# diffqc/dqc

Hardware: AMD Instinct MI355X
Metric: SCF iterations/sec (Fock build + XC grid) per GPU, cc-pVDZ 20-atom (higher is better)
Workload: dtype f64

## Files before the change

dqc_amd/csrc/jk.hip:

```cpp
#include <cstdlib>

#include "common.hpp"

namespace dqc {

DQC_DEV void decode_tri(long long t, int &a, int &b) {
    long long r = (long long)((sqrt(8.0 * (double)t + 1.0) - 1.0) * 0.5);
    while (r * (r + 1) / 2 > t) r--;
    while ((r + 1) * (r + 2) / 2 <= t) r++;
    a = (int)r;
    b = (int)(t - r * (r + 1) / 2);
}

DQC_DEV void tile_load_patch(const double *__restrict__ tiles, int IJ, int KL, int I, int J, int K, int L, int r0, int c0, double2 &a0, double2 &b0, double2 &a1, double2 &b1, double2 &a2,
                             double2 &b2, double2 &a3, double2 &b3, const TileLay &ly) {
    const bool dr = I == J, dc = K == L;
    const double *tp = tiles + tile_base(I, J, K, KL, ly);
    const bool trunc = I == ly.last && ly.wl < 8;
    if (!dr && !dc) {
        if (trunc && r0 >= 8 * ly.wl) {
            a0 = b0 = a1 = b1 = a2 = b2 = a3 = b3 = make_double2(0.0, 0.0);
            return;
        }
        const double *q = tp + r0 * 64 + c0;
        a0 = *reinterpret_cast<const double2 *>(q);       b0 = *reinterpret_cast<const double2 *>(q + 2);
        a1 = *reinterpret_cast<const double2 *>(q + 64);  b1 = *reinterpret_cast<const double2 *>(q + 66);
        a2 = *reinterpret_cast<const double2 *>(q + 128); b2 = *reinterpret_cast<const double2 *>(q + 130);
        a3 = *reinterpret_cast<const double2 *>(q + 192); b3 = *reinterpret_cast<const double2 *>(q + 194);
        return;
    }
    const int il = r0 >> 3, j0 = r0 & 7, kl = c0 >> 3, l0 = c0 & 7;
    const double2 z2 = make_double2(0.0, 0.0);
    const bool ok0 = !trunc || (dr ? max(il, j0) < ly.wl : il < ly.wl), ok1 = !trunc || (dr ? max(il, j0 + 1) < ly.wl : il < ly.wl);
    const bool ok2 = !trunc || (dr ? max(il, j0 + 2) < ly.wl : il < ly.wl), ok3 = !trunc || (dr ? max(il, j0 + 3) < ly.wl : il < ly.wl);
    if (!dc) {
        const double *q0 = tp + tile_pidx(true, il, j0) * 64 + c0, *q1 = tp + tile_pidx(true, il, j0 + 1) * 64 + c0;
        const double *q2 = tp + tile_pidx(true, il, j0 + 2) * 64 + c0, *q3 = tp + tile_pidx(true, il, j0 + 3) * 64 + c0;
        a0 = b0 = a1 = b1 = a2 = b2 = a3 = b3 = z2;
        if (ok0) { a0 = *reinterpret_cast<const double2 *>(q0); b0 = *reinterpret_cast<const double2 *>(q0 + 2); }
        if (ok1) { a1 = *reinterpret_cast<const double2 *>(q1); b1 = *reinterpret_cast<const double2 *>(q1 + 2); }
        if (ok2) { a2 = *reinterpret_cast<const double2 *>(q2); b2 = *reinterpret_cast<const double2 *>(q2 + 2); }
        if (ok3) { a3 = *reinterpret_cast<const double2 *>(q3); b3 = *reinterpret_cast<const double2 *>(q3 + 2); }
        return;
    }
    const int C = 36;
    const int pc0 = tile_pidx(dc, kl, l0), pc1 = tile_pidx(dc, kl, l0 + 1), pc2 = tile_pidx(dc, kl, l0 + 2), pc3 = tile_pidx(dc, kl, l0 + 3);
    const double *q0 = tp + tile_pidx(dr, il, j0) * C, *q1 = tp + tile_pidx(dr, il, j0 + 1) * C;
    const double *q2 = tp + tile_pidx(dr, il, j0 + 2) * C, *q3 = tp + tile_pidx(dr, il, j0 + 3) * C;
    a0 = b0 = a1 = b1 = a2 = b2 = a3 = b3 = z2;
    if (ok0) { a0 = make_double2(q0[pc0], q0[pc1]); b0 = make_double2(q0[pc2], q0[pc3]); }
    if (ok1) { a1 = make_double2(q1[pc0], q1[pc1]); b1 = make_double2(q1[pc2], q1[pc3]); }
    if (ok2) { a2 = make_double2(q2[pc0], q2[pc1]); b2 = make_double2(q2[pc2], q2[pc3]); }
    if (ok3) { a3 = make_double2(q3[pc0], q3[pc1]); b3 = make_double2(q3[pc2], q3[pc3]); }
}

__global__ void jk_prep_kernel(double *__restrict__ work, const double *__restrict__ dm, int nao, int npad, int with_k) {
    const size_t n2 = (size_t)npad * npad;
    for (size_t e = (size_t)blockIdx.x * blockDim.x + threadIdx.x; e < n2; e += (size_t)gridDim.x * blockDim.x) {
        const int i = e / npad, j = e % npad;
        double v = 0.0;
        if (i < nao && j < nao) v = 0.5 * (dm[(size_t)i * nao + j] + dm[(size_t)j * nao + i]);
        work[e] = v;
        work[n2 + e] = 0.0;
        if (with_k) work[2 * n2 + e] = 0.0;
    }
}

__global__ void jk_finish_kernel(double *__restrict__ J, double *__restrict__ K, const double *__restrict__ work,
                                 int nao, int npad, const double *__restrict__ dscp) {
    const double dsc = dscp ? *dscp : 0.0;
    const size_t n2 = (size_t)npad * npad;
    const size_t tot = (size_t)nao * nao;
    for (size_t e = (size_t)blockIdx.x * blockDim.x + threadIdx.x; e < tot; e += (size_t)gridDim.x * blockDim.x) {
        const int i = e / nao, j = e % nao;
        J[e] = det_value(work[n2 + (size_t)i * npad + j], dsc) + det_value(work[n2 + (size_t)j * npad + i], dsc);
        if (K) K[e] = det_value(work[2 * n2 + (size_t)i * npad + j], dsc) + det_value(work[2 * n2 + (size_t)j * npad + i], dsc);
    }
}

__global__ __launch_bounds__(256) void jk_det_scale_kernel(double *__restrict__ slot, const double *__restrict__ dms, int nmat,
                                                           size_t n2, const double *__restrict__ tiles, int nao) {
    __shared__ double red[256];
    const int t = threadIdx.x;
    double smax = 0.0;
    for (int q = 0; q < nmat; q++) {
        double sacc = 0.0;
        for (size_t e = t; e < n2; e += 256) sacc += fabs(dms[q * n2 + e]);
        red[t] = sacc;
        __syncthreads();
        for (int o = 128; o > 0; o >>= 1) {
            if (t < o) red[t] += red[t + o];
            __syncthreads();
        }
        smax = fmax(smax, red[0]);
        __syncthreads();
    }
    double g = 0.0;
    for (int i = t; i < nao; i += 256) {
        const long long b = i >> 3, IJ = b * (b + 1) / 2 + b;
        const int pa = tile_pidx(true, i & 7, i & 7);
        g = fmax(g, fabs(tiles[tile_base((int)b, (int)b, (int)b, (int)IJ, TileLay(nao)) + pa * 36 + pa]));
    }
    red[t] = g;
    __syncthreads();
    for (int o = 128; o > 0; o >>= 1) {
        if (t < o) red[t] = fmax(red[t], red[t + o]);
        __syncthreads();
    }
    if (t == 0) {
        const double bound = 2.0 * fmax(red[0], 1e-300) * fmax(smax, 1e-300);
        slot[0] = exp2(floor(61.0 - log2(bound)));
    }
}

template <int NK>
__global__ __launch_bounds__(256, NK ? 3 : 1) void jk_multi_kernel(const double *__restrict__ dscp, const double *__restrict__ tiles,
                                                                   double *__restrict__ work, int npad, long long ntiles, int nj, int nao) {
    const TileLay ly(nao);
    const double dsc = dscp ? *dscp : 0.0;
    constexpr int LDT = 68;
    constexpr int NKD = NK ? NK : 1;
    __shared__ double s_col[2][4][64];
    __shared__ __attribute__((aligned(16))) double s_g[NK ? 64 * LDT : 2];
    __shared__ __attribute__((aligned(16))) double s_d[4][72][NKD];
    const size_t n2 = (size_t)npad * npad;
    const double *Dj = work, *Dk = work + (size_t)nj * n2;
    double *Jacc = work + (size_t)(nj + NK) * n2, *Kacc = Jacc + (size_t)nj * n2;
    const int t = threadIdx.x, lane = t & 63, wave = t >> 6;
    const int r0 = 4 * (t >> 4), c0 = 4 * (t & 15);
    typedef double vd2 __attribute__((ext_vector_type(2)));

    double2 na0, na1, na2, na3, nb0, nb1, nb2, nb3;
#define JKM_LOAD(TT)                                                                     \
    {                                                                                    \
        int ij_, kl_, i_, j_, k_, l_;                                                    \
        decode_tri((TT), ij_, kl_);                                                      \
        decode_tri(ij_, i_, j_);                                                         \
        decode_tri(kl_, k_, l_);                                                         \
        tile_load_patch(tiles, ij_, kl_, i_, j_, k_, l_, r0, c0, na0, nb0, na1, nb1, na2, nb2, na3, nb3, ly); \
    }
    if ((long long)blockIdx.x < ntiles) JKM_LOAD(blockIdx.x)
    for (long long T = blockIdx.x; T < ntiles; T += gridDim.x) {
        int IJ, KL, I, J, K, L;
        decode_tri(T, IJ, KL);
        decode_tri(IJ, I, J);
        decode_tri(KL, K, L);
        const double f = (I == J ? 0.5 : 1.0) * (K == L ? 0.5 : 1.0) * (IJ == KL ? 0.5 : 1.0);
        const int kk = c0 >> 3, l0 = c0 & 7, ii = r0 >> 3, j0 = r0 & 7;
        double g[4][4];
        g[0][0] = na0.x; g[0][1] = na0.y; g[0][2] = nb0.x; g[0][3] = nb0.y;
        g[1][0] = na1.x; g[1][1] = na1.y; g[1][2] = nb1.x; g[1][3] = nb1.y;
        g[2][0] = na2.x; g[2][1] = na2.y; g[2][2] = nb2.x; g[2][3] = nb2.y;
        g[3][0] = na3.x; g[3][1] = na3.y; g[3][2] = nb3.x; g[3][3] = nb3.y;
        if (T + gridDim.x < ntiles) JKM_LOAD(T + gridDim.x)
        if (NK) {
#pragma unroll
            for (int r = 0; r < 4; r++) {
                *reinterpret_cast<double2 *>(&s_g[(r0 + r) * LDT + c0]) = make_double2(g[r][0], g[r][1]);
                *reinterpret_cast<double2 *>(&s_g[(r0 + r) * LDT + c0 + 2]) = make_double2(g[r][2], g[r][3]);
            }
            const int blk = t >> 6, e = t & 63, x = e >> 3, y = e & 7;
            const int R = (blk & 1) ? I : J, Cb = (blk & 2) ? L : K;
#pragma unroll
            for (int q = 0; q < NK; q++) s_d[blk][x * 9 + y][q] = Dk[q * n2 + (size_t)(R * 8 + x) * npad + Cb * 8 + y];
        }
        for (int q = 0; q < nj; q++) {
            const double *dklp = Dj + q * n2 + (size_t)(K * 8 + kk) * npad + L * 8 + l0;
            const double *dijp = Dj + q * n2 + (size_t)(I * 8 + ii) * npad + J * 8 + j0;
            double dkl[4], dij[4];
#pragma unroll
            for (int c = 0; c < 4; c++) { dkl[c] = dklp[c]; dij[c] = dijp[c]; }
            double rs[4] = {0, 0, 0, 0}, cs[4] = {0, 0, 0, 0};
#pragma unroll
            for (int r = 0; r < 4; r++)
#pragma unroll
                for (int c = 0; c < 4; c++) {
                    rs[r] += g[r][c] * dkl[c];
                    cs[c] += g[r][c] * dij[r];
                }
#pragma unroll
            for (int r = 0; r < 4; r++) {
                double v = rs[r];
                v += __shfl_xor(v, 1); v += __shfl_xor(v, 2); v += __shfl_xor(v, 4); v += __shfl_xor(v, 8);
                rs[r] = v;
            }
#pragma unroll
            for (int c = 0; c < 4; c++) {
                double v = cs[c];
                v += __shfl_xor(v, 16); v += __shfl_xor(v, 32);
                cs[c] = v;
            }
            double *Jq = Jacc + q * n2;
            if ((lane & 15) == 0) {
#pragma unroll
                for (int r = 0; r < 4; r++) acc_add(&Jq[(size_t)(I * 8 + ii) * npad + J * 8 + j0 + r], 2.0 * f * rs[r], dsc);
            }
            if (lane < 16) {
#pragma unroll
                for (int c = 0; c < 4; c++) s_col[q & 1][wave][c0 + c] = cs[c];
            }
            __syncthreads();
            if (t < 64) {
                const double v = s_col[q & 1][0][t] + s_col[q & 1][1][t] + s_col[q & 1][2][t] + s_col[q & 1][3][t];
                acc_add(&Jq[(size_t)(K * 8 + (t >> 3)) * npad + L * 8 + (t & 7)], 2.0 * f * v, dsc);
            }
        }
        if (NK) {
            if (nj == 0) __syncthreads();
            const int o = t >> 2, pg = t & 3, x = o >> 3, y = o & 7, yh = y >> 2;
            double k1[NKD], k2[NKD], k3[NKD], k4[NKD];
#pragma unroll
            for (int q = 0; q < NK; q++) k1[q] = k2[q] = k3[q] = k4[q] = 0.0;
#pragma unroll 1
            for (int u = 0; u < 2; u++) {
                const int qq = pg + 4 * u, q4 = pg + 4 * (u ^ yh);
#pragma unroll 4
                for (int a = 0; a < 8; a++) {
                    const double g1 = s_g[(x * 8 + a) * LDT + qq * 8 + y], g2 = s_g[(a * 8 + x) * LDT + qq * 8 + y];
                    const double g3 = s_g[(x * 8 + a) * LDT + y * 8 + q4], g4 = s_g[(a * 8 + x) * LDT + y * 8 + q4];
                    if constexpr (NK == 2) {
                        const vd2 d1 = *reinterpret_cast<const vd2 *>(&s_d[0][a * 9 + qq][0]);
                        const vd2 d2 = *reinterpret_cast<const vd2 *>(&s_d[1][a * 9 + qq][0]);
                        const vd2 d3 = *reinterpret_cast<const vd2 *>(&s_d[2][a * 9 + q4][0]);
                        const vd2 d4 = *reinterpret_cast<const vd2 *>(&s_d[3][a * 9 + q4][0]);
                        k1[0] += g1 * d1.x; k1[1] += g1 * d1.y;
                        k2[0] += g2 * d2.x; k2[1] += g2 * d2.y;
                        k3[0] += g3 * d3.x; k3[1] += g3 * d3.y;
                        k4[0] += g4 * d4.x; k4[1] += g4 * d4.y;
                    } else {
#pragma unroll
                        for (int q = 0; q < NK; q++) {
                            k1[q] += g1 * s_d[0][a * 9 + qq][q];
                            k2[q] += g2 * s_d[1][a * 9 + qq][q];
                            k3[q] += g3 * s_d[2][a * 9 + q4][q];
                            k4[q] += g4 * s_d[3][a * 9 + q4][q];
                        }
                    }
                }
            }
#pragma unroll
            for (int q = 0; q < NK; q++) {
                double a1 = k1[q], a2 = k2[q], a3 = k3[q], a4 = k4[q];
                a1 += __shfl_xor(a1, 1); a1 += __shfl_xor(a1, 2);
                a2 += __shfl_xor(a2, 1); a2 += __shfl_xor(a2, 2);
                a3 += __shfl_xor(a3, 1); a3 += __shfl_xor(a3, 2);
                a4 += __shfl_xor(a4, 1); a4 += __shfl_xor(a4, 2);
                if (pg == 0) {
                    double *Kq = Kacc + q * n2;
                    acc_add(&Kq[(size_t)(I * 8 + x) * npad + L * 8 + y], f * a1, dsc);
                    acc_add(&Kq[(size_t)(J * 8 + x) * npad + L * 8 + y], f * a2, dsc);
                    acc_add(&Kq[(size_t)(I * 8 + x) * npad + K * 8 + y], f * a3, dsc);
                    acc_add(&Kq[(size_t)(J * 8 + x) * npad + K * 8 + y], f * a4, dsc);
                }
            }
        }
        __syncthreads();
    }
}

#undef JKM_LOAD
__global__ void jk_multi_prep_kernel(double *__restrict__ work, const double *__restrict__ dmj, int nj, const double *__restrict__ dmk,
                                     int nk, int nao, int npad, unsigned kanti) {
    const size_t n2 = (size_t)npad * npad, nn = (size_t)nao * nao;
    const int nd = nj + nk;
    for (size_t e = (size_t)blockIdx.x * blockDim.x + threadIdx.x; e < n2 * nd; e += (size_t)gridDim.x * blockDim.x) {
        const int q = e / n2;
        const size_t r = e - (size_t)q * n2;
        const int i = r / npad, j = r % npad;
        const double *dm = q < nj ? dmj + (size_t)q * nn : dmk + (size_t)(q - nj) * nn;
        double v = 0.0;
        const bool anti = q >= nj && ((kanti >> (q - nj)) & 1u);
        if (i < nao && j < nao) v = anti ? 0.5 * (dm[(size_t)i * nao + j] - dm[(size_t)j * nao + i]) : 0.5 * (dm[(size_t)i * nao + j] + dm[(size_t)j * nao + i]);
        work[e] = v;
        work[n2 * nd + e] = 0.0;
    }
}

__global__ void jk_multi_finish_kernel(double *__restrict__ J, int nj, double *__restrict__ K, int nk, const double *__restrict__ work,
                                       int nao, int npad, const double *__restrict__ dscp, unsigned kanti) {
    const double dsc = dscp ? *dscp : 0.0;
    const size_t n2 = (size_t)npad * npad, nn = (size_t)nao * nao;
    const double *acc = work + (size_t)(nj + nk) * n2;
    for (size_t e = (size_t)blockIdx.x * blockDim.x + threadIdx.x; e < nn * (nj + nk); e += (size_t)gridDim.x * blockDim.x) {
        const int q = e / nn;
        const size_t r = e - (size_t)q * nn;
        const int i = r / nao, j = r % nao;
        const double a = det_value(acc[q * n2 + (size_t)i * npad + j], dsc), at = det_value(acc[q * n2 + (size_t)j * npad + i], dsc);
        const double v = (q >= nj && ((kanti >> (q - nj)) & 1u)) ? a - at : a + at;
        if (q < nj) J[e] = v;
        else K[e - (size_t)nj * nn] = v;
    }
}

__global__ __launch_bounds__(256, 1) void j_stream_kernel(const double *__restrict__ dscp, const double *__restrict__ tiles,
                                                         double *__restrict__ work, int npad, long long ntiles, long long per_block,
                                                         long long tbeg, int nao) {
    const TileLay ly(nao);
    const double dsc = dscp ? *dscp : 0.0;
    __shared__ double s_col[2][4][64];
    const size_t n2 = (size_t)npad * npad;
    const double *Dp = work;
    double *Jacc = work + n2;
    const int t = threadIdx.x, lane = t & 63, wave = t >> 6;
    const int r0 = 4 * (t >> 4), c0 = 4 * (t & 15);
    const int kk = c0 >> 3, l0 = c0 & 7, ii = r0 >> 3, j0 = r0 & 7;
    const long long T0 = tbeg + (long long)blockIdx.x * per_block, T1 = min(T0 + per_block, ntiles);
    if (T0 >= T1) return;
    int IJ, KL, I, J, K, L;
    decode_tri(T0, IJ, KL);
    decode_tri(IJ, I, J);
    double rsacc[4] = {0, 0, 0, 0}, dij[4];
    {
        const double *dijp = Dp + (size_t)(I * 8 + ii) * npad + J * 8 + j0;
#pragma unroll
        for (int q = 0; q < 4; q++) dij[q] = dijp[q];
    }
    auto flush_rows = [&]() {
        const double fI = (I == J ? 0.5 : 1.0);
#pragma unroll
        for (int r = 0; r < 4; r++) {
            double v = rsacc[r];
            v += __shfl_xor(v, 1); v += __shfl_xor(v, 2); v += __shfl_xor(v, 4); v += __shfl_xor(v, 8);
            if ((lane & 15) == 0) acc_add(&Jacc[(size_t)(I * 8 + ii) * npad + J * 8 + j0 + r], 2.0 * fI * v, dsc);
            rsacc[r] = 0.0;
        }
    };
    int par = 0;
    for (long long T = T0; T < T1; T++, KL++) {
        if (KL > IJ) {
            flush_rows();
            IJ++;
            KL = 0;
            decode_tri(IJ, I, J);
            const double *dijp = Dp + (size_t)(I * 8 + ii) * npad + J * 8 + j0;
#pragma unroll
            for (int q = 0; q < 4; q++) dij[q] = dijp[q];
        }
        decode_tri(KL, K, L);
        const double fk = (K == L ? 0.5 : 1.0) * (IJ == KL ? 0.5 : 1.0);
        const double *dklp = Dp + (size_t)(K * 8 + kk) * npad + L * 8 + l0;
        double dkl[4];
#pragma unroll
        for (int q = 0; q < 4; q++) dkl[q] = fk * dklp[q];
        double cs[4] = {0, 0, 0, 0};
        {
            double2 ta0, tb0, ta1, tb1, ta2, tb2, ta3, tb3;
            tile_load_patch(tiles, IJ, KL, I, J, K, L, r0, c0, ta0, tb0, ta1, tb1, ta2, tb2, ta3, tb3, ly);
#define DQC_JS_ROW(R_, A_, B_)                                                                           \
    rsacc[R_] += A_.x * dkl[0] + A_.y * dkl[1] + B_.x * dkl[2] + B_.y * dkl[3];                          \
    cs[0] += A_.x * dij[R_]; cs[1] += A_.y * dij[R_]; cs[2] += B_.x * dij[R_]; cs[3] += B_.y * dij[R_];
            DQC_JS_ROW(0, ta0, tb0) DQC_JS_ROW(1, ta1, tb1) DQC_JS_ROW(2, ta2, tb2) DQC_JS_ROW(3, ta3, tb3)
#undef DQC_JS_ROW
        }
#pragma unroll
        for (int c = 0; c < 4; c++) {
            double v = cs[c];
            v += __shfl_xor(v, 16); v += __shfl_xor(v, 32);
            cs[c] = v;
        }
        if (lane < 16) {
#pragma unroll
            for (int c = 0; c < 4; c++) s_col[par][wave][c0 + c] = cs[c];
        }
        __syncthreads();
        if (t < 64) {
            const double v = s_col[par][0][t] + s_col[par][1][t] + s_col[par][2][t] + s_col[par][3][t];
            acc_add(&Jacc[(size_t)(K * 8 + (t >> 3)) * npad + L * 8 + (t & 7)], 2.0 * (I == J ? 0.5 : 1.0) * fk * v, dsc);
        }
        par ^= 1;
    }
    flush_rows();
}


__global__ __launch_bounds__(256, 4) void jk_stream_kernel(const double *__restrict__ dscp, const double *__restrict__ tiles,
                                                          double *__restrict__ work, int npad, long long ntiles, long long per_block,
                                                          long long tbeg, int nao) {
    const TileLay ly(nao);
    const double dsc = dscp ? *dscp : 0.0;
    constexpr int LDT = 68;
    __shared__ double s_col[4][64];
    __shared__ __attribute__((aligned(16))) double s_g[64 * LDT];
    __shared__ __attribute__((aligned(16))) double s_d[2][72][2];
    const size_t n2 = (size_t)npad * npad;
    const double *Dp = work;
    double *Jacc = work + n2, *Kacc = work + 2 * n2;
    const int t = threadIdx.x, lane = t & 63, wave = t >> 6;
    const int r0 = 4 * (t >> 4), c0 = 4 * (t & 15);
    const int kk = c0 >> 3, l0 = c0 & 7, ii = r0 >> 3, j0 = r0 & 7;
    const int o = t >> 2, pg = t & 3, x = o >> 3, y = o & 7, yh = y >> 2;
    const long long T0 = tbeg + (long long)blockIdx.x * per_block, T1 = min(T0 + per_block, ntiles);
    if (T0 >= T1) return;
    int IJ, KL, I, J, K, L;
    decode_tri(T0, IJ, KL);
    decode_tri(IJ, I, J);
    decode_tri(KL, K, L);
    double rsacc[4] = {0, 0, 0, 0}, dij[4];
    double k3acc = 0.0, k4acc = 0.0;
    {
        const double *dijp = Dp + (size_t)(I * 8 + ii) * npad + J * 8 + j0;
#pragma unroll
        for (int q = 0; q < 4; q++) dij[q] = dijp[q];
    }
    auto flush_rows = [&]() {
        const double fI = (I == J ? 0.5 : 1.0);
#pragma unroll
        for (int r = 0; r < 4; r++) {
            double v = rsacc[r];
            v += __shfl_xor(v, 1); v += __shfl_xor(v, 2); v += __shfl_xor(v, 4); v += __shfl_xor(v, 8);
            if ((lane & 15) == 0) acc_add(&Jacc[(size_t)(I * 8 + ii) * npad + J * 8 + j0 + r], 2.0 * fI * v, dsc);
            rsacc[r] = 0.0;
        }
    };
    auto flush_k34 = [&]() {
        double a3 = k3acc, a4 = k4acc;
        a3 += __shfl_xor(a3, 1); a3 += __shfl_xor(a3, 2);
        a4 += __shfl_xor(a4, 1); a4 += __shfl_xor(a4, 2);
        if (pg == 0) {
            acc_add(&Kacc[(size_t)(I * 8 + x) * npad + K * 8 + y], a3, dsc);
            acc_add(&Kacc[(size_t)(J * 8 + x) * npad + K * 8 + y], a4, dsc);
        }
        k3acc = k4acc = 0.0;
    };
    for (long long T = T0; T < T1; T++) {
        const double f = (I == J ? 0.5 : 1.0) * (K == L ? 0.5 : 1.0) * (IJ == KL ? 0.5 : 1.0);
        const double fk = (K == L ? 0.5 : 1.0) * (IJ == KL ? 0.5 : 1.0);
        const double *dklp = Dp + (size_t)(K * 8 + kk) * npad + L * 8 + l0;
        double dkl[4];
#pragma unroll
        for (int q = 0; q < 4; q++) dkl[q] = fk * dklp[q];
        double cs[4] = {0, 0, 0, 0};
        {
            double2 ta0, tb0, ta1, tb1, ta2, tb2, ta3, tb3;
            tile_load_patch(tiles, IJ, KL, I, J, K, L, r0, c0, ta0, tb0, ta1, tb1, ta2, tb2, ta3, tb3, ly);
#define DQC_JS_ROW(R_, A_, B_)                                                                           \
    rsacc[R_] += A_.x * dkl[0] + A_.y * dkl[1] + B_.x * dkl[2] + B_.y * dkl[3];                          \
    cs[0] += A_.x * dij[R_]; cs[1] += A_.y * dij[R_]; cs[2] += B_.x * dij[R_]; cs[3] += B_.y * dij[R_]; \
    *reinterpret_cast<double2 *>(&s_g[(r0 + R_) * LDT + c0]) = A_;                                       \
    *reinterpret_cast<double2 *>(&s_g[(r0 + R_) * LDT + c0 + 2]) = B_;
            DQC_JS_ROW(0, ta0, tb0) DQC_JS_ROW(1, ta1, tb1) DQC_JS_ROW(2, ta2, tb2) DQC_JS_ROW(3, ta3, tb3)
#undef DQC_JS_ROW
        }
        {
            const int blk = t >> 6, e = t & 63, xx = e >> 3, yy = e & 7;
            const int R = (blk & 1) ? I : J, Cb = (blk & 2) ? L : K;
            s_d[blk >> 1][xx * 9 + yy][blk & 1] = Dp[(size_t)(R * 8 + xx) * npad + Cb * 8 + yy];
        }
#pragma unroll
        for (int c = 0; c < 4; c++) {
            double v = cs[c];
            v += __shfl_xor(v, 16); v += __shfl_xor(v, 32);
            cs[c] = v;
        }
        if (lane < 16) {
#pragma unroll
            for (int c = 0; c < 4; c++) s_col[wave][c0 + c] = cs[c];
        }
        __syncthreads();
        if (t < 64) {
            const double v = s_col[0][t] + s_col[1][t] + s_col[2][t] + s_col[3][t];
            acc_add(&Jacc[(size_t)(K * 8 + (t >> 3)) * npad + L * 8 + (t & 7)], 2.0 * (I == J ? 0.5 : 1.0) * fk * v, dsc);
        }
        {
            double k1 = 0, k2 = 0, k3 = 0, k4 = 0;
#pragma unroll 1
            for (int u = 0; u < 2; u++) {
                const int q = pg + 4 * u, q4 = pg + 4 * (u ^ yh);
#pragma unroll
                for (int a = 0; a < 8; a++) {
                    typedef double vd2_ __attribute__((ext_vector_type(2)));
                    const vd2_ d12 = *reinterpret_cast<const vd2_ *>(&s_d[0][a * 9 + q][0]);
                    const vd2_ d34 = *reinterpret_cast<const vd2_ *>(&s_d[1][a * 9 + q4][0]);
                    k1 += s_g[(x * 8 + a) * LDT + q * 8 + y] * d12.x;
                    k2 += s_g[(a * 8 + x) * LDT + q * 8 + y] * d12.y;
                    k3 += s_g[(x * 8 + a) * LDT + y * 8 + q4] * d34.x;
                    k4 += s_g[(a * 8 + x) * LDT + y * 8 + q4] * d34.y;
                }
            }
            k1 += __shfl_xor(k1, 1); k1 += __shfl_xor(k1, 2);
            k2 += __shfl_xor(k2, 1); k2 += __shfl_xor(k2, 2);
            if (pg == 0) {
                acc_add(&Kacc[(size_t)(I * 8 + x) * npad + L * 8 + y], f * k1, dsc);
                acc_add(&Kacc[(size_t)(J * 8 + x) * npad + L * 8 + y], f * k2, dsc);
            }
            k3acc += f * k3;
            k4acc += f * k4;
        }
        if (T + 1 < T1) {
            if (KL == IJ) {
                flush_rows();
                flush_k34();
                IJ++;
                KL = 0; K = 0; L = 0;
                decode_tri(IJ, I, J);
                const double *dijp = Dp + (size_t)(I * 8 + ii) * npad + J * 8 + j0;
#pragma unroll
                for (int q = 0; q < 4; q++) dij[q] = dijp[q];
            } else {
                KL++;
                if (L == K) { flush_k34(); K++; L = 0; }
                else L++;
            }
        }
        __syncthreads();
    }
    flush_rows();
    flush_k34();
}

template <int NJ, int NK>
__global__ __launch_bounds__(256, 3) void jk_multi_stream_kernel(const double *__restrict__ dscp, const double *__restrict__ tiles,
                                                                double *__restrict__ work, int npad, long long ntiles,
                                                                long long per_block, int nao) {
    const TileLay ly(nao);
    const double dsc = dscp ? *dscp : 0.0;
    constexpr int LDT = 68;
    __shared__ double s_col[4][64];
    __shared__ __attribute__((aligned(16))) double s_g[64 * LDT];
    __shared__ __attribute__((aligned(16))) double s_d[4][72][NK];
    const size_t n2 = (size_t)npad * npad;
    const double *Dp = work, *Dk = work + (size_t)NJ * n2;
    double *Jacc = work + (size_t)(NJ + NK) * n2, *Kacc = Jacc + (size_t)NJ * n2;
    const int t = threadIdx.x, lane = t & 63, wave = t >> 6;
    const int r0 = 4 * (t >> 4), c0 = 4 * (t & 15);
    const int kk = c0 >> 3, l0 = c0 & 7, ii = r0 >> 3, j0 = r0 & 7;
    const int o = t >> 2, pg = t & 3, x = o >> 3, y = o & 7, yh = y >> 2;
    const long long T0 = (long long)blockIdx.x * per_block, T1 = min(T0 + per_block, ntiles);
    if (T0 >= T1) return;
    int IJ, KL, I, J, K, L;
    decode_tri(T0, IJ, KL);
    decode_tri(IJ, I, J);
    decode_tri(KL, K, L);
    double rsacc[4] = {0, 0, 0, 0}, dij[4];
    double k3acc[NK], k4acc[NK];
#pragma unroll
    for (int q = 0; q < NK; q++) k3acc[q] = k4acc[q] = 0.0;
    if (NJ) {
        const double *dijp = Dp + (size_t)(I * 8 + ii) * npad + J * 8 + j0;
#pragma unroll
        for (int q = 0; q < 4; q++) dij[q] = dijp[q];
    }
    auto flush_rows = [&]() {
        if (!NJ) return;
        const double fI = (I == J ? 0.5 : 1.0);
#pragma unroll
        for (int r = 0; r < 4; r++) {
            double v = rsacc[r];
            v += __shfl_xor(v, 1); v += __shfl_xor(v, 2); v += __shfl_xor(v, 4); v += __shfl_xor(v, 8);
            if ((lane & 15) == 0) acc_add(&Jacc[(size_t)(I * 8 + ii) * npad + J * 8 + j0 + r], 2.0 * fI * v, dsc);
            rsacc[r] = 0.0;
        }
    };
    auto flush_k34 = [&]() {
#pragma unroll
        for (int q = 0; q < NK; q++) {
            double a3 = k3acc[q], a4 = k4acc[q];
            a3 += __shfl_xor(a3, 1); a3 += __shfl_xor(a3, 2);
            a4 += __shfl_xor(a4, 1); a4 += __shfl_xor(a4, 2);
            if (pg == 0) {
                acc_add(&Kacc[q * n2 + (size_t)(I * 8 + x) * npad + K * 8 + y], a3, dsc);
                acc_add(&Kacc[q * n2 + (size_t)(J * 8 + x) * npad + K * 8 + y], a4, dsc);
            }
            k3acc[q] = k4acc[q] = 0.0;
        }
    };
    for (long long T = T0; T < T1; T++) {
        const double f = (I == J ? 0.5 : 1.0) * (K == L ? 0.5 : 1.0) * (IJ == KL ? 0.5 : 1.0);
        const double fk = (K == L ? 0.5 : 1.0) * (IJ == KL ? 0.5 : 1.0);
        const double *dklp = Dp + (size_t)(K * 8 + kk) * npad + L * 8 + l0;
        double dkl[4];
#pragma unroll
        for (int q = 0; q < 4; q++) dkl[q] = NJ ? fk * dklp[q] : 0.0;
        double cs[4] = {0, 0, 0, 0};
        {
            double2 ta0, tb0, ta1, tb1, ta2, tb2, ta3, tb3;
            tile_load_patch(tiles, IJ, KL, I, J, K, L, r0, c0, ta0, tb0, ta1, tb1, ta2, tb2, ta3, tb3, ly);
#define DQC_JS_ROW(R_, A_, B_)                                                                           \
    if (NJ) {                                                                                            \
        rsacc[R_] += A_.x * dkl[0] + A_.y * dkl[1] + B_.x * dkl[2] + B_.y * dkl[3];                      \
        cs[0] += A_.x * dij[R_]; cs[1] += A_.y * dij[R_]; cs[2] += B_.x * dij[R_]; cs[3] += B_.y * dij[R_]; \
    }                                                                                                    \
    *reinterpret_cast<double2 *>(&s_g[(r0 + R_) * LDT + c0]) = A_;                                       \
    *reinterpret_cast<double2 *>(&s_g[(r0 + R_) * LDT + c0 + 2]) = B_;
            DQC_JS_ROW(0, ta0, tb0) DQC_JS_ROW(1, ta1, tb1) DQC_JS_ROW(2, ta2, tb2) DQC_JS_ROW(3, ta3, tb3)
#undef DQC_JS_ROW
        }
        {
            const int blk = t >> 6, e = t & 63, xx = e >> 3, yy = e & 7;
            const int R = (blk & 1) ? I : J, Cb = (blk & 2) ? L : K;
#pragma unroll
            for (int q = 0; q < NK; q++) s_d[blk][xx * 9 + yy][q] = Dk[q * n2 + (size_t)(R * 8 + xx) * npad + Cb * 8 + yy];
        }
        if (NJ) {
#pragma unroll
            for (int c = 0; c < 4; c++) {
                double v = cs[c];
                v += __shfl_xor(v, 16); v += __shfl_xor(v, 32);
                cs[c] = v;
            }
            if (lane < 16) {
#pragma unroll
                for (int c = 0; c < 4; c++) s_col[wave][c0 + c] = cs[c];
            }
        }
        __syncthreads();
        if (NJ && t < 64) {
            const double v = s_col[0][t] + s_col[1][t] + s_col[2][t] + s_col[3][t];
            acc_add(&Jacc[(size_t)(K * 8 + (t >> 3)) * npad + L * 8 + (t & 7)], 2.0 * (I == J ? 0.5 : 1.0) * fk * v, dsc);
        }
        {
            double k1[NK], k2[NK], k3[NK], k4[NK];
#pragma unroll
            for (int q = 0; q < NK; q++) k1[q] = k2[q] = k3[q] = k4[q] = 0.0;
#pragma unroll 1
            for (int u = 0; u < 2; u++) {
                const int qq = pg + 4 * u, q4 = pg + 4 * (u ^ yh);
#pragma unroll 4
                for (int a = 0; a < 8; a++) {
                    const double g1 = s_g[(x * 8 + a) * LDT + qq * 8 + y], g2 = s_g[(a * 8 + x) * LDT + qq * 8 + y];
                    const double g3 = s_g[(x * 8 + a) * LDT + y * 8 + q4], g4 = s_g[(a * 8 + x) * LDT + y * 8 + q4];
#pragma unroll
                    for (int q = 0; q < NK; q++) {
                        k1[q] += g1 * s_d[0][a * 9 + qq][q];
                        k2[q] += g2 * s_d[1][a * 9 + qq][q];
                        k3[q] += g3 * s_d[2][a * 9 + q4][q];
                        k4[q] += g4 * s_d[3][a * 9 + q4][q];
                    }
                }
            }
#pragma unroll
            for (int q = 0; q < NK; q++) {
                double a1 = k1[q], a2 = k2[q];
                a1 += __shfl_xor(a1, 1); a1 += __shfl_xor(a1, 2);
                a2 += __shfl_xor(a2, 1); a2 += __shfl_xor(a2, 2);
                if (pg == 0) {
                    acc_add(&Kacc[q * n2 + (size_t)(I * 8 + x) * npad + L * 8 + y], f * a1, dsc);
                    acc_add(&Kacc[q * n2 + (size_t)(J * 8 + x) * npad + L * 8 + y], f * a2, dsc);
                }
                k3acc[q] += f * k3[q];
                k4acc[q] += f * k4[q];
            }
        }
        if (T + 1 < T1) {
            if (KL == IJ) {
                flush_rows();
                flush_k34();
                IJ++;
                KL = 0; K = 0; L = 0;
                decode_tri(IJ, I, J);
                if (NJ) {
                    const double *dijp = Dp + (size_t)(I * 8 + ii) * npad + J * 8 + j0;
#pragma unroll
                    for (int q = 0; q < 4; q++) dij[q] = dijp[q];
                }
            } else {
                KL++;
                if (L == K) { flush_k34(); K++; L = 0; }
                else L++;
            }
        }
        __syncthreads();
    }
    flush_rows();
    flush_k34();
}


}

extern "C" {

size_t dqc_jk_work_doubles(int nao) {
    const size_t npad = (size_t)(nao + DQC_TILE_B - 1) / DQC_TILE_B * DQC_TILE_B;
    return 5 * npad * npad + 8 + 128;
}

long long dqc_eri_tile_offset(int nao, long long tile) {
    using namespace dqc;
    const long long nt = (long long)dqc_eri_tile_count(nao);
    if (nao <= 0 || tile <= 0) return 0;
    if (tile >= nt) return eri_store_data_doubles(nao);
    auto tri = [](long long t, long long &a, long long &b) {
        long long r = (long long)((std::sqrt(8.0 * (double)t + 1.0) - 1.0) * 0.5);
        while (r * (r + 1) / 2 > t) r--;
        while ((r + 1) * (r + 2) / 2 <= t) r++;
        a = r;
        b = t - r * (r + 1) / 2;
    };
    long long IJ, KL, I, J, K, L;
    tri(tile, IJ, KL);
    tri(IJ, I, J);
    tri(KL, K, L);
    return tile_base((int)I, (int)J, (int)K, (int)KL, TileLay(nao));
}

int dqc_jk_from_tiles(double *d_J, double *d_K, const double *d_tiles, const double *d_dm, int nao,
                      double *d_work, void *stream) {
    return dqc_jk_from_tiles_part(d_J, d_K, d_tiles, d_dm, nao, d_work, 0, (long long)dqc_eri_tile_count(nao), stream);
}

static int jk_from_tiles_impl(double *d_J, double *d_K, const double *d_tiles_part, const double *d_dm, int nao, double *d_work,
                              long long tile_begin, long long tile_end, int with_k_prepared, void *stream);

int dqc_jk_from_tiles_part(double *d_J, double *d_K, const double *d_tiles_part, const double *d_dm, int nao, double *d_work,
                           long long tile_begin, long long tile_end, void *stream) {
    return jk_from_tiles_impl(d_J, d_K, d_tiles_part, d_dm, nao, d_work, tile_begin, tile_end, 0, stream);
}

int dqc_jk_stream_prepared(const double *d_tiles, int nao, double *d_work, int with_k, void *stream) {
    return jk_from_tiles_impl(nullptr, nullptr, d_tiles, nullptr, nao, d_work, 0, (long long)dqc_eri_tile_count(nao), with_k ? 1 : 0, stream);
}

static int jk_from_tiles_impl(double *d_J, double *d_K, const double *d_tiles_part, const double *d_dm, int nao, double *d_work,
                              long long tile_begin, long long tile_end, int with_k_prepared, void *stream) {
    using namespace dqc;
    if (nao <= 0) return DQC_OK;
    hipStream_t st = (hipStream_t)stream;
    const int npad = (nao + DQC_TILE_B - 1) / DQC_TILE_B * DQC_TILE_B;
    const long long nt_all = (long long)dqc_eri_tile_count(nao);
    if (tile_begin < 0 || tile_end > nt_all || tile_begin > tile_end) { set_error("dqc_jk_from_tiles_part: tile range outside the store"); return DQC_EINVAL; }
    const bool whole = tile_begin == 0 && tile_end == nt_all;
    if (!whole && deterministic_mode()) {
        set_error("dqc_jk_from_tiles_part: the deterministic mode needs the whole store (its scale reads the diagonal tiles)");
        return DQC_EINVAL;
    }
    const double *d_tiles = d_tiles_part - dqc_eri_tile_offset(nao, tile_begin);
    const long long ntiles = tile_end, tbeg = tile_begin, nrun = tile_end - tile_begin;
    const int with_k = d_dm ? (d_K != nullptr) : with_k_prepared;
    if (d_dm) {
        hipLaunchKernelGGL(jk_prep_kernel, dim3(64), dim3(256), 0, st, d_work, d_dm, nao, npad, with_k);
        DQC_CHECK_LAUNCH();
    }
    double *dscp = nullptr;
    if (deterministic_mode()) {
        dscp = d_work + 3 * (size_t)npad * npad;
        hipLaunchKernelGGL(jk_det_scale_kernel, dim3(1), dim3(256), 0, st, dscp, d_work, 1, (size_t)npad * npad, d_tiles, nao);
        DQC_CHECK_LAUNCH();
    }
    if (nrun == 0) {
    } else if (with_k) {
        static const long long jk_nblk_env = [] { const char *e = getenv("DQC_JK_NBLK"); return e ? atoll(e) : 0LL; }();
        const long long nblk = jk_nblk_env > 0 ? std::min<long long>(nrun, jk_nblk_env) : std::min<long long>(nrun, std::max<long long>(1024, std::min<long long>(6144, nrun / 8)));
        const long long per = (nrun + nblk - 1) / nblk;
        hipLaunchKernelGGL(jk_stream_kernel, dim3((unsigned)((nrun + per - 1) / per)), dim3(256), 0, st, dscp, d_tiles, d_work, npad, ntiles, per, tbeg, nao);
    } else {
        static const long long j_nblk_env = [] { const char *e = getenv("DQC_J_NBLK"); return e ? atoll(e) : 0LL; }();
        const long long nblk = std::max<long long>(1, std::min<long long>((nrun + 3) / 4, j_nblk_env > 0 ? j_nblk_env : 65536));
        const long long per = (nrun + nblk - 1) / nblk;
        hipLaunchKernelGGL(j_stream_kernel, dim3((unsigned)((nrun + per - 1) / per)), dim3(256), 0, st, dscp, d_tiles, d_work, npad, ntiles, per, tbeg, nao);
    }
    DQC_CHECK_LAUNCH();
    if (d_J) {
        hipLaunchKernelGGL(jk_finish_kernel, dim3(64), dim3(256), 0, st, d_J, d_K, d_work, nao, npad, dscp);
        DQC_CHECK_LAUNCH();
    }
    return DQC_OK;
}

size_t dqc_jk_multi_work_doubles(int nao, int nj, int nk) {
    const size_t npad = (size_t)(nao + DQC_TILE_B - 1) / DQC_TILE_B * DQC_TILE_B;
    return 2 * (size_t)(nj + (nk > 2 ? 2 : nk)) * npad * npad + 8;
}

static int jk_from_tiles_multi_impl(double *d_J, const double *d_dmJ, int nj, double *d_K, const double *d_dmK, int nk, const int *k_antisym,
                                    const double *d_tiles, int nao, double *d_work, void *stream);

int dqc_jk_from_tiles_multi(double *d_J, const double *d_dmJ, int nj, double *d_K, const double *d_dmK, int nk,
                            const double *d_tiles, int nao, double *d_work, void *stream) {
    return jk_from_tiles_multi_impl(d_J, d_dmJ, nj, d_K, d_dmK, nk, nullptr, d_tiles, nao, d_work, stream);
}

int dqc_jk_from_tiles_multi_asym(double *d_J, const double *d_dmJ, int nj, double *d_K, const double *d_dmK, int nk, const int *k_antisym,
                                 const double *d_tiles, int nao, double *d_work, void *stream) {
    return jk_from_tiles_multi_impl(d_J, d_dmJ, nj, d_K, d_dmK, nk, k_antisym, d_tiles, nao, d_work, stream);
}

static int jk_from_tiles_multi_impl(double *d_J, const double *d_dmJ, int nj, double *d_K, const double *d_dmK, int nk, const int *k_antisym,
                                    const double *d_tiles, int nao, double *d_work, void *stream) {
    using namespace dqc;
    if (nao <= 0 || (nj <= 0 && nk <= 0)) return DQC_OK;
    if (nj < 0 || nk < 0) { set_error("dqc_jk_from_tiles_multi: negative matrix count"); return DQC_EINVAL; }
    hipStream_t st = (hipStream_t)stream;
    const int npad = (nao + DQC_TILE_B - 1) / DQC_TILE_B * DQC_TILE_B;
    const size_t nn = (size_t)nao * nao;
    const long long ntiles = (long long)dqc_eri_tile_count(nao);
    const unsigned grid = (unsigned)std::min<long long>(ntiles, 256 * 16);
    int kdone = 0, first = 1;
    while (first || kdone < nk) {
        const int njp = first ? nj : 0, nkp = std::min(2, nk - kdone);
        unsigned kanti = 0;
        for (int q = 0; k_antisym && q < nkp; q++) kanti |= k_antisym[kdone + q] ? 1u << q : 0u;
        hipLaunchKernelGGL(jk_multi_prep_kernel, dim3(64), dim3(256), 0, st, d_work, d_dmJ, njp, d_dmK + (size_t)kdone * nn, nkp, nao, npad, kanti);
        DQC_CHECK_LAUNCH();
        double *dscp = nullptr;
        if (deterministic_mode()) {
            dscp = d_work + 2 * (size_t)(njp + nkp) * npad * npad;
            hipLaunchKernelGGL(jk_det_scale_kernel, dim3(1), dim3(256), 0, st, dscp, d_work, njp + nkp, (size_t)npad * npad, d_tiles, nao);
            DQC_CHECK_LAUNCH();
        }
        const long long nblk_s = std::min<long long>(ntiles, std::max<long long>(1024, std::min<long long>(6144, ntiles / 8)));
        const long long per_s = (ntiles + nblk_s - 1) / nblk_s;
        const dim3 grid_s((unsigned)((ntiles + per_s - 1) / per_s));
        const bool stream_ok = njp <= 1 && nkp >= 1;
        if (stream_ok && njp == 1 && nkp == 2) hipLaunchKernelGGL((jk_multi_stream_kernel<1, 2>), grid_s, dim3(256), 0, st, dscp, d_tiles, d_work, npad, ntiles, per_s, nao);
        else if (stream_ok && njp == 1 && nkp == 1) hipLaunchKernelGGL((jk_multi_stream_kernel<1, 1>), grid_s, dim3(256), 0, st, dscp, d_tiles, d_work, npad, ntiles, per_s, nao);
        else if (stream_ok && njp == 0 && nkp == 2) hipLaunchKernelGGL((jk_multi_stream_kernel<0, 2>), grid_s, dim3(256), 0, st, dscp, d_tiles, d_work, npad, ntiles, per_s, nao);
        else if (stream_ok && njp == 0 && nkp == 1) hipLaunchKernelGGL((jk_multi_stream_kernel<0, 1>), grid_s, dim3(256), 0, st, dscp, d_tiles, d_work, npad, ntiles, per_s, nao);
        else if (nkp == 2) hipLaunchKernelGGL(jk_multi_kernel<2>, dim3(grid), dim3(256), 0, st, dscp, d_tiles, d_work, npad, ntiles, njp, nao);
        else if (nkp == 1) hipLaunchKernelGGL(jk_multi_kernel<1>, dim3(grid), dim3(256), 0, st, dscp, d_tiles, d_work, npad, ntiles, njp, nao);
        else hipLaunchKernelGGL(jk_multi_kernel<0>, dim3(grid), dim3(256), 0, st, dscp, d_tiles, d_work, npad, ntiles, njp, nao);
        DQC_CHECK_LAUNCH();
        hipLaunchKernelGGL(jk_multi_finish_kernel, dim3(64), dim3(256), 0, st, d_J, njp, d_K + (size_t)kdone * nn, nkp, d_work, nao, npad, dscp, kanti);
        DQC_CHECK_LAUNCH();
        kdone += nkp;
        first = 0;
    }
    return DQC_OK;
}

}
```

Baseline: 800.2.

## Software-pipeline tile loads in J stream kernel with double-buffered register tiles

Restructures the J-only streaming kernel so each tile's ERI patch and D(kl) values are fetched one iteration ahead into a second register set (JTile A/B ping-pong), overlapping global loads with the FMA and reduction work of the current tile. Tile indices are made wave-uniform via readfirstlane, loads are made unconditional with clamped offsets and row masks applied during compute, and the diagonal K==L case reloads through a dedicated packed path. Launch bounds are raised from 1 to 3 blocks per CU for more occupancy. The cost is higher register pressure from two in-flight tiles, plus redundant loads for the K==L case.

```diff
diff --git a/dqc_amd/csrc/jk.hip b/dqc_amd/csrc/jk.hip
--- a/dqc_amd/csrc/jk.hip
+++ b/dqc_amd/csrc/jk.hip
@@ -10,6 +10,12 @@
     while ((r + 1) * (r + 2) / 2 <= t) r++;
     a = (int)r;
     b = (int)(t - r * (r + 1) / 2);
+}
+
+DQC_DEV void decode_tri_u(long long t, int &a, int &b) {
+    decode_tri(t, a, b);
+    a = __builtin_amdgcn_readfirstlane(a);
+    b = __builtin_amdgcn_readfirstlane(b);
 }
 
 DQC_DEV void tile_load_patch(const double *__restrict__ tiles, int IJ, int KL, int I, int J, int K, int L, int r0, int c0, double2 &a0, double2 &b0, double2 &a1, double2 &b1, double2 &a2,
@@ -53,6 +59,54 @@
     if (ok2) { a2 = make_double2(q2[pc0], q2[pc1]); b2 = make_double2(q2[pc2], q2[pc3]); }
     if (ok3) { a3 = make_double2(q3[pc0], q3[pc1]); b3 = make_double2(q3[pc2], q3[pc3]); }
 }
+
+typedef double jk_v2d __attribute__((ext_vector_type(2)));
+DQC_DEV double2 tile_ld2(const double *p) {
+    const jk_v2d v = *reinterpret_cast<const jk_v2d *>(p);
+    return make_double2(v.x, v.y);
+}
+DQC_DEV unsigned tile_issue_patch(const double *__restrict__ tiles, int KL, int I, int J, int K, int L, int t, int r0, int c0, double2 &a0, double2 &b0, double2 &a1, double2 &b1,
+                                  double2 &a2, double2 &b2, double2 &a3, double2 &b3, const TileLay &ly) {
+    const bool dr = I == J, dc = K == L;
+    const double *tp = tiles + tile_base(I, J, K, KL, ly);
+    const bool trunc = I == ly.last && ly.wl < 8;
+    const int il = r0 >> 3, j0 = r0 & 7;
+    const bool ok0 = !trunc || (dr ? max(il, j0) < ly.wl : il < ly.wl), ok1 = !trunc || (dr ? max(il, j0 + 1) < ly.wl : il < ly.wl);
+    const bool ok2 = !trunc || (dr ? max(il, j0 + 2) < ly.wl : il < ly.wl), ok3 = !trunc || (dr ? max(il, j0 + 3) < ly.wl : il < ly.wl);
+    const unsigned last4 = tile_rows(I, J, ly) * 36 - 4;
+    const unsigned o0 = dc ? min(4u * t, last4) : (ok0 ? tile_pidx(dr, il, j0) : 0) * 64 + c0;
+    const unsigned o1 = dc ? min(4u * t + 1024u, last4) : (ok1 ? tile_pidx(dr, il, j0 + 1) : 0) * 64 + c0;
+    const unsigned o2 = dc ? min(4u * t + 2048u, last4) : (ok2 ? tile_pidx(dr, il, j0 + 2) : 0) * 64 + c0;
+    const unsigned o3 = dc ? last4 : (ok3 ? tile_pidx(dr, il, j0 + 3) : 0) * 64 + c0;
+    a0 = tile_ld2(tp + o0); b0 = tile_ld2(tp + o0 + 2);
+    a1 = tile_ld2(tp + o1); b1 = tile_ld2(tp + o1 + 2);
+    a2 = tile_ld2(tp + o2); b2 = tile_ld2(tp + o2 + 2);
+    a3 = tile_ld2(tp + o3); b3 = tile_ld2(tp + o3 + 2);
+    return dc ? 15u : (ok0 ? 1u : 0u) | (ok1 ? 2u : 0u) | (ok2 ? 4u : 0u) | (ok3 ? 8u : 0u);
+}
+DQC_DEV void tile_load_patch_kk(const double *__restrict__ tiles, int KL, int I, int J, int K, int r0, int c0, double2 &a0, double2 &b0, double2 &a1, double2 &b1, double2 &a2,
+                                double2 &b2, double2 &a3, double2 &b3, const TileLay &ly) {
+    const bool dr = I == J;
+    const double *tp = tiles + tile_base(I, J, K, KL, ly);
+    const bool trunc = I == ly.last && ly.wl < 8;
+    const int il = r0 >> 3, j0 = r0 & 7, kl = c0 >> 3, l0 = c0 & 7;
+    const double2 z2 = make_double2(0.0, 0.0);
+    const bool ok0 = !trunc || (dr ? max(il, j0) < ly.wl : il < ly.wl), ok1 = !trunc || (dr ? max(il, j0 + 1) < ly.wl : il < ly.wl);
+    const bool ok2 = !trunc || (dr ? max(il, j0 + 2) < ly.wl : il < ly.wl), ok3 = !trunc || (dr ? max(il, j0 + 3) < ly.wl : il < ly.wl);
+    const unsigned pc0 = tile_pidx(true, kl, l0), pc1 = tile_pidx(true, kl, l0 + 1), pc2 = tile_pidx(true, kl, l0 + 2), pc3 = tile_pidx(true, kl, l0 + 3);
+    const unsigned q0 = tile_pidx(dr, il, j0) * 36u, q1 = tile_pidx(dr, il, j0 + 1) * 36u, q2 = tile_pidx(dr, il, j0 + 2) * 36u, q3 = tile_pidx(dr, il, j0 + 3) * 36u;
+    a0 = b0 = a1 = b1 = a2 = b2 = a3 = b3 = z2;
+    if (ok0) { a0 = make_double2(tp[q0 + pc0], tp[q0 + pc1]); b0 = make_double2(tp[q0 + pc2], tp[q0 + pc3]); }
+    if (ok1) { a1 = make_double2(tp[q1 + pc0], tp[q1 + pc1]); b1 = make_double2(tp[q1 + pc2], tp[q1 + pc3]); }
+    if (ok2) { a2 = make_double2(tp[q2 + pc0], tp[q2 + pc1]); b2 = make_double2(tp[q2 + pc2], tp[q2 + pc3]); }
+    if (ok3) { a3 = make_double2(tp[q3 + pc0], tp[q3 + pc1]); b3 = make_double2(tp[q3 + pc2], tp[q3 + pc3]); }
+}
+struct JTile {
+    double2 a0, b0, a1, b1, a2, b2, a3, b3;
+    double d0, d1, d2, d3;
+    int IJ, KL, I, J, K, L;
+    unsigned rows;
+};
 
 __global__ void jk_prep_kernel(double *__restrict__ work, const double *__restrict__ dm, int nao, int npad, int with_k) {
     const size_t n2 = (size_t)npad * npad;
@@ -292,7 +346,7 @@
     }
 }
 
-__global__ __launch_bounds__(256, 1) void j_stream_kernel(const double *__restrict__ dscp, const double *__restrict__ tiles,
+__global__ __launch_bounds__(256, 3) void j_stream_kernel(const double *__restrict__ dscp, const double *__restrict__ tiles,
                                                          double *__restrict__ work, int npad, long long ntiles, long long per_block,
                                                          long long tbeg, int nao) {
     const TileLay ly(nao);
@@ -306,16 +360,18 @@
     const int kk = c0 >> 3, l0 = c0 & 7, ii = r0 >> 3, j0 = r0 & 7;
     const long long T0 = tbeg + (long long)blockIdx.x * per_block, T1 = min(T0 + per_block, ntiles);
     if (T0 >= T1) return;
-    int IJ, KL, I, J, K, L;
-    decode_tri(T0, IJ, KL);
-    decode_tri(IJ, I, J);
+    int IJ, I, J, pIJ, pKL, pI, pJ;
+    decode_tri_u(T0, pIJ, pKL);
+    decode_tri_u(pIJ, pI, pJ);
+    IJ = pIJ; I = pI; J = pJ;
     double rsacc[4] = {0, 0, 0, 0}, dij[4];
-    {
+    auto load_dij = [&]() __attribute__((always_inline)) {
         const double *dijp = Dp + (size_t)(I * 8 + ii) * npad + J * 8 + j0;
 #pragma unroll
         for (int q = 0; q < 4; q++) dij[q] = dijp[q];
-    }
-    auto flush_rows = [&]() {
+    };
+    load_dij();
+    auto flush_rows = [&]() __attribute__((always_inline)) {
         const double fI = (I == J ? 0.5 : 1.0);
 #pragma unroll
         for (int r = 0; r < 4; r++) {
@@ -325,33 +381,55 @@
             rsacc[r] = 0.0;
         }
     };
-    int par = 0;
-    for (long long T = T0; T < T1; T++, KL++) {
-        if (KL > IJ) {
+    auto advance = [&]() __attribute__((always_inline)) {
+        if (++pKL > pIJ) {
+            pIJ++;
+            pKL = 0;
+            decode_tri_u(pIJ, pI, pJ);
+        }
+    };
+    auto issue = [&](JTile &X) __attribute__((always_inline)) {
+        X.IJ = pIJ; X.KL = pKL; X.I = pI; X.J = pJ;
+        decode_tri_u(pKL, X.K, X.L);
+        const double *dklp = Dp + (size_t)(X.K * 8 + kk) * npad + X.L * 8 + l0;
+        X.d0 = dklp[0]; X.d1 = dklp[1]; X.d2 = dklp[2]; X.d3 = dklp[3];
+        int r0i = r0, c0i = c0;
+        asm volatile("" : "+v"(r0i), "+v"(c0i));
+        X.rows = tile_issue_patch(tiles, X.KL, X.I, X.J, X.K, X.L, t, r0i, c0i, X.a0, X.b0, X.a1, X.b1, X.a2, X.b2, X.a3, X.b3, ly);
+        __builtin_amdgcn_sched_barrier(0);
+    };
+    auto turn = [&](const JTile &X) __attribute__((always_inline)) {
+        if (X.IJ != IJ) {
             flush_rows();
-            IJ++;
-            KL = 0;
-            decode_tri(IJ, I, J);
-            const double *dijp = Dp + (size_t)(I * 8 + ii) * npad + J * 8 + j0;
-#pragma unroll
-            for (int q = 0; q < 4; q++) dij[q] = dijp[q];
-        }
-        decode_tri(KL, K, L);
-        const double fk = (K == L ? 0.5 : 1.0) * (IJ == KL ? 0.5 : 1.0);
-        const double *dklp = Dp + (size_t)(K * 8 + kk) * npad + L * 8 + l0;
-        double dkl[4];
-#pragma unroll
-        for (int q = 0; q < 4; q++) dkl[q] = fk * dklp[q];
+            IJ = X.IJ; I = X.I; J = X.J;
+            load_dij();
+        }
+    };
+    auto consume = [&](const JTile &X, const int par) __attribute__((always_inline)) {
+        const double fk = (X.K == X.L ? 0.5 : 1.0) * (X.IJ == X.KL ? 0.5 : 1.0);
+        const double dkl[4] = {fk * X.d0, fk * X.d1, fk * X.d2, fk * X.d3};
         double cs[4] = {0, 0, 0, 0};
-        {
-            double2 ta0, tb0, ta1, tb1, ta2, tb2, ta3, tb3;
-            tile_load_patch(tiles, IJ, KL, I, J, K, L, r0, c0, ta0, tb0, ta1, tb1, ta2, tb2, ta3, tb3, ly);
-#define DQC_JS_ROW(R_, A_, B_)                                                                           \
-    rsacc[R_] += A_.x * dkl[0] + A_.y * dkl[1] + B_.x * dkl[2] + B_.y * dkl[3];                          \
-    cs[0] += A_.x * dij[R_]; cs[1] += A_.y * dij[R_]; cs[2] += B_.x * dij[R_]; cs[3] += B_.y * dij[R_];
-            DQC_JS_ROW(0, ta0, tb0) DQC_JS_ROW(1, ta1, tb1) DQC_JS_ROW(2, ta2, tb2) DQC_JS_ROW(3, ta3, tb3)
+#define DQC_JS_ROW(R_, A_, B_, IN_)                                                                      \
+    {                                                                                                    \
+        const bool in = (IN_);                                                                           \
+        const double k0 = in ? dkl[0] : 0.0, k1 = in ? dkl[1] : 0.0, k2 = in ? dkl[2] : 0.0, k3 = in ? dkl[3] : 0.0; \
+        const double dj = in ? dij[R_] : 0.0;                                                            \
+        rsacc[R_] += fma(B_.y, k3, fma(B_.x, k2, fma(A_.y, k1, A_.x * k0)));                              \
+        cs[0] = fma(A_.x, dj, cs[0]); cs[1] = fma(A_.y, dj, cs[1]); cs[2] = fma(B_.x, dj, cs[2]); cs[3] = fma(B_.y, dj, cs[3]); \
+    }
+        if (X.K == X.L) {
+            asm volatile("" ::"v"(X.a0.x), "v"(X.a0.y), "v"(X.b0.x), "v"(X.b0.y), "v"(X.a1.x), "v"(X.a1.y), "v"(X.b1.x), "v"(X.b1.y), "v"(X.a2.x),
+                         "v"(X.a2.y), "v"(X.b2.x), "v"(X.b2.y), "v"(X.a3.x), "v"(X.a3.y), "v"(X.b3.x), "v"(X.b3.y));
+            int r0d = r0, c0d = c0;
+            asm volatile("" : "+v"(r0d), "+v"(c0d));
+            double2 pa0, pb0, pa1, pb1, pa2, pb2, pa3, pb3;
+            tile_load_patch_kk(tiles, X.KL, X.I, X.J, X.K, r0d, c0d, pa0, pb0, pa1, pb1, pa2, pb2, pa3, pb3, ly);
+            DQC_JS_ROW(0, pa0, pb0, true) DQC_JS_ROW(1, pa1, pb1, true) DQC_JS_ROW(2, pa2, pb2, true) DQC_JS_ROW(3, pa3, pb3, true)
+        } else {
+            DQC_JS_ROW(0, X.a0, X.b0, X.rows & 1u) DQC_JS_ROW(1, X.a1, X.b1, X.rows & 2u)
+            DQC_JS_ROW(2, X.a2, X.b2, X.rows & 4u) DQC_JS_ROW(3, X.a3, X.b3, X.rows & 8u)
+        }
 #undef DQC_JS_ROW
-        }
 #pragma unroll
         for (int c = 0; c < 4; c++) {
             double v = cs[c];
@@ -365,9 +443,20 @@
         __syncthreads();
         if (t < 64) {
             const double v = s_col[par][0][t] + s_col[par][1][t] + s_col[par][2][t] + s_col[par][3][t];
-            acc_add(&Jacc[(size_t)(K * 8 + (t >> 3)) * npad + L * 8 + (t & 7)], 2.0 * (I == J ? 0.5 : 1.0) * fk * v, dsc);
-        }
-        par ^= 1;
+            acc_add(&Jacc[(size_t)(X.K * 8 + (t >> 3)) * npad + X.L * 8 + (t & 7)], 2.0 * (I == J ? 0.5 : 1.0) * fk * v, dsc);
+        }
+    };
+    JTile A, B;
+    issue(A);
+    for (long long T = T0;; T += 2) {
+        if (T + 1 >= T1) { consume(A, 0); break; }
+        advance(); issue(B);
+        consume(A, 0);
+        turn(B);
+        if (T + 2 >= T1) { consume(B, 1); break; }
+        advance(); issue(A);
+        consume(B, 1);
+        turn(A);
     }
     flush_rows();
 }
```

New measurement: 803.8, median of 6. Within noise of the previous version (+0.4%).
